# tridivb/attention_based_tbn

Hardware: AMD Instinct MI355X
Metric: clips/sec (3-seg RGB+Flow+Audio TBN fwd+bwd) (higher is better)
Workload: dtype f32; 1 GPU; BASELINE config 4: RGB+Flow+Audio async, attention off, 3 segments, 224x224 frames + 1.279 s (256x256) spectrogram, train step fwd+loss+bwd+clip+SGD; batch_per_gpu=32, global_batch=32, segments=3, parallelism=single, launch_plans=committed (bench_plans.json)

## Files before the change

### attention_based_tbn_amd/_lib.py

```python
import ctypes as C
import os

_HERE = os.path.dirname(os.path.abspath(__file__))
LIB_PATH = os.path.join(_HERE, "libtbn_hip.so")
if os.environ.get("TBN_LIB"):
    import sys as _sys
    LIB_PATH = os.path.abspath(os.environ["TBN_LIB"])
    print(f"[tbn] TBN_LIB set: loading {LIB_PATH} instead of the shipped libtbn_hip.so", file=_sys.stderr)

c_fp = C.c_void_p
c_i = C.c_int
c_sz = C.c_size_t
c_f = C.c_float


class ConvInfo(C.Structure):
    _fields_ = [("name", C.c_char * 64), ("cin", c_i), ("cout", c_i), ("ksize", c_i), ("stride", c_i),
                ("pad", c_i), ("weight_offset", c_sz), ("channel_offset", c_sz)]


class BackboneParams(C.Structure):
    _fields_ = [("weight", c_fp), ("bias", c_fp), ("gamma", c_fp), ("beta", c_fp), ("running_mean", c_fp),
                ("running_var", c_fp), ("momentum", c_f), ("eps", c_f), ("side_stream", c_fp), ("flags", c_i),
                ("weight_planes", c_fp)]
# ... 83 lines not shown
    "tbn_bn_relu_train_bwd": (c_i, [c_fp, c_i, c_fp, c_i, c_i, c_fp, c_fp, c_fp, c_fp, c_fp, c_fp, c_fp, c_fp, c_fp]),
    "tbn_bn_relu_maxpool_train_fwd": (c_i, [c_fp, c_i, c_i, c_i, c_i, c_fp, c_fp, c_fp, c_fp, c_f, c_f, c_fp, c_fp, c_fp,
                                            c_fp, c_fp, c_i, c_fp, c_i, c_i, c_i, c_i, c_fp, c_fp]),
    "tbn_bn_relu_maxpool_train_bwd": (c_i, [c_fp, c_i, c_fp, c_fp, c_i, c_i, c_i, c_i, c_i, c_i, c_i, c_i, c_fp, c_fp,
                                            c_fp, c_fp, c_fp, c_fp, c_fp, c_fp, c_fp]),
    "tbn_maxpool3_fwd": (c_i, [c_fp, c_i, c_fp, c_i, c_fp] + [c_i] * 8 + [c_fp]),
    "tbn_maxpool3_bwd": (c_i, [c_fp, c_i, c_fp, c_fp, c_i] + [c_i] * 9 + [c_fp]),
    "tbn_avgpool3_fwd": (c_i, [c_fp, c_i, c_fp, c_i] + [c_i] * 5 + [c_fp]),
    "tbn_spatial_mean_fwd": (c_i, [c_fp, c_i, c_fp, c_i] + [c_i] * 5 + [c_fp]),
    "tbn_spatial_mean_bwd": (c_i, [c_fp, c_i, c_fp, c_i] + [c_i] * 5 + [c_fp]),
    "tbn_pe_concat_fwd": (c_i, [c_fp, c_i, c_fp, c_fp, c_i, c_i, c_i, c_i, c_i, c_fp]),
    "tbn_groupnorm_fwd": (c_i, [c_fp, c_fp, c_fp, c_fp, c_fp, c_fp, c_i, c_i, c_i, c_i, c_f, c_fp]),
    "tbn_groupnorm_bwd": (c_i, [c_fp] * 8 + [c_i] * 4 + [c_fp]),
    "tbn_colsum": (c_i, [c_fp, c_i, c_fp, c_i, c_i, c_fp]),
    "tbn_mha_q1_fwd": (c_i, [c_fp] * 6 + [c_i] * 4 + [c_f, c_fp]),
    "tbn_mha_q1_bwd": (c_i, [c_fp] * 8 + [c_i] * 4 + [c_f, c_fp]),
    "tbn_weighted_sum_fwd": (c_i, [c_fp, c_fp, c_fp, c_i, c_i, c_i, c_i, c_fp]),
    "tbn_weighted_sum_bwd": (c_i, [c_fp, c_i, c_fp, c_fp, c_i, c_i, c_i, c_fp]),
    "tbn_segment_mean_fwd": (c_i, [c_fp, c_fp, c_i, c_i, c_i, c_fp]),
    "tbn_segment_mean_bwd": (c_i, [c_fp, c_fp, c_i, c_i, c_i, c_fp]),
    "tbn_dropout_fwd": (c_i, [c_fp, c_fp, c_f, c_fp, c_fp, c_sz, c_fp]),
    "tbn_ce_heads_fwd": (c_i, [c_fp, c_i, c_i, c_i, C.POINTER(c_i), C.POINTER(c_i), C.POINTER(C.c_void_p), c_fp, c_fp, c_fp, c_fp]),
    "tbn_ce_heads_bwd": (c_i, [c_fp, c_i, c_i, c_i, C.POINTER(c_i), C.POINTER(c_i), c_fp, c_fp, c_fp]),
    "tbn_mul_mask": (c_i, [c_fp, c_fp, c_fp, c_sz, c_fp]),
    "tbn_relu_mask_bwd": (c_i, [c_fp, c_fp, c_fp, c_fp, c_sz, c_fp]),
    "tbn_stft_twiddle_floats": (c_sz, []),
    "tbn_stft_make_twiddle": (c_i, [c_fp]),
    "tbn_stft_logpower": (c_i, [c_fp, c_i, c_i, c_fp, c_fp, c_f, c_fp]),
    "tbn_opt_num_partials": (c_i, [C.POINTER(OptTensor), c_i]),
    "tbn_opt_sqnorm_partials": (c_i, [C.POINTER(OptTensor), c_i, c_fp, c_fp]),
    "tbn_opt_clip_coef": (c_i, [c_fp, c_i, c_f, c_fp, c_fp, c_fp]),
    "tbn_opt_scale_grads": (c_i, [C.POINTER(OptTensor), c_i, c_fp, c_fp]),
    "tbn_opt_sgd_step": (c_i, [C.POINTER(OptTensor), c_i, c_f, c_f, c_f, c_fp, c_fp]),
    "tbn_topk_correct": (c_i, [c_fp, c_i, c_fp, c_i, c_i, c_i, c_fp, c_fp, c_fp, c_fp]),
    "tbn_frames_to_tensor": (c_i, [c_fp] + [c_i] * 16 + [c_fp, c_fp, c_i, c_i, c_fp, c_fp]),
}

_lib = None


class TbnHipError(RuntimeError):
    pass


def lib():
    global _lib
# ... 47 lines not shown
```

### attention_based_tbn_amd/core/models/model.py

```python
import os
import weakref
from collections import OrderedDict

import numpy as np
import torch
import torch.nn as nn
from torch.distributions import Categorical

from ... import ops
from .attention import MultiheadedAttention, PositionalEncoding, PrototypeAttention, UniModalAttention
from .bn_inception import bninception


class _ArenaCatFn(torch.autograd.Function):

    @staticmethod
    def forward(ctx, arena, *feats):
        ctx.widths = [f.shape[1] for f in feats]
        return arena.detach()

    @staticmethod
    def backward(ctx, g):
        out, o = [], 0
        for w in ctx.widths:
# ... 46 lines not shown
        return ops.group_norm(y.view(R, T, -1), gn.weight, gn.bias, gn.num_groups, gn.eps)

    def forward(self, x):
        return self.forward_sequence(x.squeeze(2).transpose(1, 2).contiguous()).transpose(1, 2)


class TBNModel(nn.Module):
    IN_CHANNELS = {"RGB": 3, "Flow": 10, "Audio": 1}

    def __init__(self, cfg, modality, device, pretrained_state=None):
        super().__init__()
        self.cfg = cfg
        self.modality = modality
        self.base_model_name = cfg.model.arch
        self.num_classes = cfg.model.num_classes
        self.use_attention = cfg.model.attention.enable
        self.attention_type = cfg.model.attention.type
        self.device = device
        self._pretrained_state = pretrained_state
        self.multi_stream = True
        self._streams = {}
        self.high_priority_modalities = ("Audio",)
        self.flip_weights_early = True
        self.shared_streams = {}
        if cfg.model.agg_type.lower() == "avg":
            self.agg_type = "avg"
        else:
            print("Incorrect aggregation type")
            self.agg_type = None

        in_features = 0
        for m in self.modality:
            self.add_module("Base_{}".format(m), self._create_base_model(m))
            in_features += getattr(self, "Base_{}".format(m)).feature_size
            getattr(self, "Base_{}".format(m)).use_aux_stream = len(self.modality) == 1
            getattr(self, "Base_{}".format(m)).use_branch_streams = len(self.modality) == 1
            getattr(self, "Base_{}".format(m)).stem_wgrad_last = len(self.modality) > 1
            if cfg.model.freeze_base:
                self._freeze_base_model(m, freeze_mode=cfg.model.freeze_mode)

        if len(self.modality) > 1:
            att = cfg.model.attention
            if self.use_attention and not att.use_fixed:
                attn_win_size = round(self.cfg.data.audio.audio_length * (25 / 4))
                if att.use_pe:
                    self.pe = _PEStack(PositionalEncoding(10, max_len=attn_win_size, device=device),
# ... 92 lines not shown
    def _run_backbones_inner(self, input):
        def run(m):
            b, n, c, h, w = input[m].shape
            base = getattr(self, "Base_{}".format(m))
            x = input[m].reshape(b * n, c, h, w)
            return base.forward_sequence(x) if (m == "Audio" and self.use_attention) else base(x)

        first = input[self.modality[0]]
        if not (self.multi_stream and first.is_cuda and len(self.modality) > 1):
            return {m: run(m) for m in self.modality}
        main = torch.cuda.current_stream()
        raw = {}
        share = self.shared_streams
        for m in self.modality:
            if m in share and share[m] in self._streams:
                self._streams[m] = self._streams[share[m]]
            st = self._streams.get(m)
            if st is None or st.device != first.device:
                st = self._streams[m] = torch.cuda.Stream(device=first.device,
                                                          priority=(-1 if m in self.high_priority_modalities else 0))
            st.wait_stream(main)
            with torch.cuda.stream(st):
                raw[m] = run(m)
        for m in self.modality:
            main.wait_stream(self._streams[m])
            raw[m].record_stream(main)
        if self.flip_weights_early and torch.is_grad_enabled():
            for m in self.modality:
                with torch.cuda.stream(self._streams[m]):
                    getattr(self, "Base_{}".format(m)).flip_weights_early()
        return raw

    def forward(self, input):
        features = []
        att_wts = None
        att = self.cfg.model.attention
        self._audio_dropped = False
        raw_all = self._run_backbones(input)
        for m_no, m in enumerate(self.modality):
            b, n, c, h, w = input[m].shape
            if m == "Audio":
                raw = raw_all[m]
                if (self.training and len(self.modality) > 1 and self.cfg.data.audio.dropout > 0
                        and np.random.uniform() > self.cfg.data.audio.dropout):
                    feature = torch.zeros_like(features[0])
                    self._audio_dropped = True
                elif self.use_attention:
                    seq = raw
                    if att.use_fixed:
                        feature = ops.weighted_sum(seq, input["weights"].reshape(b * n, -1).to(seq.device))
                    elif self.attention_type == "mha":
                        seq = self.pe.forward_sequence(seq)
                        feature, att_wts = self.attention_layer.attend(features[0], seq)
                        att_wts = att_wts.unsqueeze(1)
                    elif self.attention_type in ["unimodal", "proto"]:
                        feature, att_wts = self.attention_layer.attend(features[0], seq)
                else:
                    feature = raw
                if m_no > 0 and features[0].shape[0] > feature.shape[0]:
                    new_size = features[0].shape[0] // feature.shape[0]
                    feature = feature.repeat(new_size, 1)
                    n *= new_size
            else:
                feature = raw_all[m]
            features.extend([feature])
        if len(features) > 1:
            features = _concat_features(self._arena, features)
        else:
            features = features[0]
        self._arena = None

        if len(self.modality) > 1:
            features = self.fusion(features)

        out = self.classifier(features, consensus=(b, n))

        if self.use_attention and not att.use_fixed and len(self.modality) > 1:
            if att_wts is None:
                raise UnboundLocalError("local variable 'att_wts' referenced before assignment (audio dropout with a "
                                        "trainable attention layer: the reference fails the same way)")
            out["weights"] = att_wts
        return out

    def _fused_cross_entropy(self, criterion, target, preds):
        ce = criterion.get("crossentropy")
        keys = list(target["class"].keys())
        if (type(ce) is not nn.CrossEntropyLoss or ce.weight is not None or ce.ignore_index != -100
                or ce.reduction != "mean" or getattr(ce, "label_smoothing", 0.0) != 0.0 or not 1 <= len(keys) <= 4):
            return None
        shared = self.classifier.shared_scores(preds, keys)
        if shared is None:
            return None
        base, heads = shared
        labels = []
        for k in keys:
            lab = target["class"][k]
            if (not base.is_cuda or not torch.is_tensor(lab) or not lab.is_cuda or lab.dtype != torch.int64 or lab.dim() != 1
                    or lab.shape[0] != base.shape[0]):
                return None
            labels.append(lab)
        return dict(zip(keys, ops.cross_entropy_heads(base, heads, labels)))

    def get_loss(self, criterion, target, preds, epoch=0):
        assert isinstance(target, dict)
        assert isinstance(preds, dict)
        assert isinstance(criterion, dict)
        att = self.cfg.model.attention
        loss = {"total": 0, "all_class": 0}
        fused = self._fused_cross_entropy(criterion, target, preds) if hasattr(self, "classifier") else None
        for key in target["class"].keys():
            labels = target["class"][key]
            batch_size = target["class"][key].shape[0]
            loss[key] = fused[key] if fused is not None else criterion["crossentropy"](preds[key], labels)
            loss["all_class"] += loss[key]
        loss["total"] += loss["all_class"]

        if self.use_attention and not att.use_fixed:
            if self.training and epoch + 1 < att.decay_step:
                prior_multiplier = contrast_multiplier = entropy_multiplier = 0
            else:
                prior_multiplier = att.wt_decay
                contrast_multiplier = att.contrast_decay
                entropy_multiplier = att.entropy_decay
# ... 20 lines not shown
class Fusion(nn.Module):

    def __init__(self, in_size, out_size, dropout=0):
        super().__init__()
        self.in_size, self.out_size, self.dropout = in_size, out_size, dropout
        self.fusion_layer = nn.Sequential(nn.Linear(in_size, out_size), nn.ReLU())
        torch.nn.init.normal_(self.fusion_layer[0].weight, 0, 1e-3)
        torch.nn.init.constant_(self.fusion_layer[0].bias, 0)
        if self.dropout > 0:
            self.dropout_layer = nn.Dropout(p=self.dropout)

    def forward(self, input):
        lin = self.fusion_layer[0]
        out = ops.linear(input, lin.weight, lin.bias, relu=True)
        return ops.dropout(out, self.dropout, self.training)


class Classifier(nn.Module):

    def __init__(self, num_classes, in_features):
        super().__init__()
        self.num_classes = num_classes
        self._wcache, self._bcache = {}, {}
        for cls in num_classes.keys():
            self.add_module(cls, nn.Linear(in_features, self.num_classes[cls]))
            torch.nn.init.normal_(getattr(self, cls).weight, 0, 1e-3)
            torch.nn.init.constant_(getattr(self, cls).bias, 0)

    def forward(self, input, consensus=None):
        keys = list(self.num_classes.keys())
        w = ops.cat_pad_rows(self._wcache, 32, *[getattr(self, k).weight for k in keys])
        b = ops.cat_pad_rows(self._bcache, 32, *[getattr(self, k).bias for k in keys])
        scores = ops.linear(input, w, b)
        if consensus is not None:
            scores = ops.segment_mean(scores, consensus[0], consensus[1])
        out = OrderedDict()
        layout = {}
        o = 0
        for k in keys:
            out[k] = scores[:, o:o + self.num_classes[k]].contiguous()
            layout[k] = (weakref.ref(out[k]), o, self.num_classes[k], out[k]._version)
            o += self.num_classes[k]
        self._shared = (scores, layout)
        return out

    def shared_scores(self, preds, keys):
        shared = getattr(self, "_shared", None)
        if shared is None:
            return None
        scores, layout = shared
        heads = []
        for k in keys:
            ent = layout.get(k)
            t = preds.get(k) if hasattr(preds, "get") else None
            if ent is None or t is None or ent[0]() is not t or t._version != ent[3] or not scores.is_contiguous():
                return None
            heads.append((ent[1], ent[2]))
        return scores, heads
```

### attention_based_tbn_amd/csrc/api.hip

```cpp
#include <cstdarg>
#include <cstdio>
#include <cstdlib>
#include <cstring>

#include "tbn_common.h"
#include "tbn_kernels.h"
#include "../../include/tbn_hip.h"

static thread_local char g_err[512] = "";

void tbn_set_error(const char* fmt, ...) {
  va_list ap;
  va_start(ap, fmt);
  vsnprintf(g_err, sizeof(g_err), fmt, ap);
  va_end(ap);
}

#if TBN_EXPERIMENT
int tbn_env_int(const char* name, int def, int lo, int hi) {
  const char* e = getenv(name);
  if (e == nullptr || *e == 0) return def;
  char* end = nullptr;
  const long v = strtol(e, &end, 10);
  if (end == e || *end != 0 || v < lo || v > hi) {
// ... 208 lines not shown
  g_prof_open = -1;
}

__global__ __launch_bounds__(256) void mfma_burst_kernel(float* sink, int iters) {
  f32x16 a0, a1, a2, a3;
#pragma unroll
  for (int e = 0; e < 16; ++e) a0[e] = a1[e] = a2[e] = a3[e] = 0.f;
  const float x = 1e-3f * (float)(threadIdx.x & 63) + 0.5f, y = 1.0f - 1e-3f * (float)(threadIdx.x >> 6);
  for (int i = 0; i < iters; ++i) {
#pragma unroll
    for (int k = 0; k < 4; ++k) {
      a0 = __builtin_amdgcn_mfma_f32_32x32x2f32(x, y, a0, 0, 0, 0);
      a1 = __builtin_amdgcn_mfma_f32_32x32x2f32(y, x, a1, 0, 0, 0);
      a2 = __builtin_amdgcn_mfma_f32_32x32x2f32(x, x, a2, 0, 0, 0);
      a3 = __builtin_amdgcn_mfma_f32_32x32x2f32(y, y, a3, 0, 0, 0);
    }
  }
  float s = 0.f;
#pragma unroll
  for (int e = 0; e < 16; ++e) s += (a0[e] + a1[e]) + (a2[e] + a3[e]);
  if (s == -1.2345f) sink[0] = s;
}

extern "C" {

int tbn_version(void) { return 102 | (TBN_EXPERIMENT ? 0x10000 : 0); }

int tbn_capabilities(void) { return TBN_CAP_CONV_BF16X | TBN_CAP_CONV_BF16X_PLANES; }

int tbn_diag_mfma_burst(float* sink, int workgroups, int iters, double* flops, void* stream) {
  TBN_REQUIRE(sink != nullptr && workgroups > 0 && workgroups <= 65536 && iters > 0, "diag_mfma_burst: bad argument");
  hipLaunchKernelGGL(mfma_burst_kernel, dim3(workgroups), dim3(256), 0, (hipStream_t)stream, sink, iters);
  TBN_CHECK_LAUNCH("mfma_burst");
  if (flops) *flops = (double)workgroups * 4.0 * (double)iters * 16.0 * 4096.0;
  return TBN_OK;
}

int tbn_profile_enable(int on) {
  std::lock_guard<std::mutex> lk(g_prof_mu);
  g_prof_on = on != 0;
  g_prof_layers = on == 2;
  return TBN_OK;
}
int tbn_profile_reset(void) {
  std::lock_guard<std::mutex> lk(g_prof_mu);
  prof_collect();
// ... 64 lines not shown
                        float* stat_partial, int mt, int nt, void* stream) {
  ConvP p;
  conv_geom(&p, n, h, w, cin, cout, ksize, stride, pad);
  p.in = in;
  p.in_ld = in_ld;
  p.wt = weight;
  p.bias = bias;
  p.stat_partial = stat_partial;
  p.mode = epilogue;
  p.flags = flags;
  p.nseg = 1;
  p.seg[0].ptr = out;
  p.seg[0].ld = out_ld;
  p.seg[0].col_begin = 0;
  return tbn_launch_conv(p, 0, mt, nt, (hipStream_t)stream);
}

int tbn_conv2d_dgrad(const float* dout, int dout_ld, const float* weight, float* din, int din_ld, int n, int h, int w,
                     int cin, int cout, int ksize, int stride, int pad, int accumulate, float* workspace,
                     void* stream) {
  TBN_REQUIRE(dout && weight && din && workspace, "conv2d_dgrad: null pointer");
  hipStream_t st = (hipStream_t)stream;
  TBN_TRY(tbn_launch_weight_flip_transpose(weight, workspace, cout, ksize * ksize, cin, st));
  const int oh = (h + 2 * pad - ksize) / stride + 1, ow = (w + 2 * pad - ksize) / stride + 1;
  ConvP p;
  memset(&p, 0, sizeof(p));
  p.in = dout;
  p.in_ld = dout_ld;
  p.wt = workspace;
  p.N = n;
  p.H = oh;
  p.W = ow;
  p.OH = h;
  p.OW = w;
  p.Cin = cout;
  p.Cout = cin;
  p.R = p.S = ksize;
  p.stride = 1;
  p.pad = ksize - 1 - pad;
  p.up = stride;
  p.M = n * h * w;
  p.K = ksize * ksize * cout;
  p.mode = CONV_EPI_PLAIN;
  p.flags = accumulate ? CONV_FLAG_ACCUM : 0;
  p.nseg = 1;
  p.seg[0].ptr = din;
  p.seg[0].ld = din_ld;
  p.seg[0].col_begin = 0;
  return tbn_launch_conv(p, 0, 0, 0, st);
}

static int desc_to_convp(const tbn_conv_desc* d, float* workspace, hipStream_t st, ConvP* pp) {
  ConvP& p = *pp;
  TBN_REQUIRE(d && d->in && d->weight && d->out, "conv_launch: null pointer");
  if (!d->dgrad) {
    TBN_REQUIRE(d->epilogue >= 0 && d->epilogue <= 2, "conv_launch: bad epilogue");
    TBN_REQUIRE(d->epilogue != CONV_EPI_STATS || d->stat_partial, "conv_launch: stats epilogue needs stat_partial");
    TBN_REQUIRE(d->epilogue != CONV_EPI_EVAL || (d->scale && d->shift), "conv_launch: eval epilogue needs scale/shift");
    TBN_REQUIRE(d->nred == 0, "conv_launch: the fused BN-backward reduce belongs to a data gradient");
    conv_geom(&p, d->n, d->h, d->w, d->cin, d->cout, d->ksize, d->stride, d->pad);
    p.in = d->in;
    p.in_ld = d->in_ld;
    p.wt = d->weight;
    p.bias = d->bias;
    p.scale = d->scale;
    p.shift = d->shift;
    p.stat_partial = d->stat_partial;
    p.mode = d->epilogue;
  } else {
    if (d->flags & (CONV_FLAG_BF16X6 | CONV_FLAG_BF16X3 | CONV_FLAG_BF16X_PLANES)) {
      tbn_set_error("conv_launch: the bf16x kernels (flags 32 / 64) compute forward convolutions only, not dgrad = 1");
      return TBN_ERR_UNSUPPORTED;
    }
// ... 138 lines not shown
int tbn_linear_fwd(const float* x, int x_ld, const float* w, const float* bias, float* out, int out_ld, int m, int k,
                   int n, int relu, void* stream) {
  ProfPrefix scope("linear: ");
  return tbn_conv2d_fwd(x, x_ld, w, bias, out, out_ld, m, 1, 1, k, n, 1, 1, 0, CONV_EPI_PLAIN,
                        relu ? CONV_FLAG_RELU : 0, nullptr, nullptr, nullptr, stream);
}

int tbn_linear_dgrad(const float* dy, int dy_ld, const float* w, float* dx, int dx_ld, int m, int k, int n,
                     int accumulate, float* workspace, void* stream) {
  ProfPrefix scope("linear: ");
  return tbn_conv2d_dgrad(dy, dy_ld, w, dx, dx_ld, m, 1, 1, k, n, 1, 1, 0, accumulate, workspace, stream);
}

size_t tbn_linear_wgrad_workspace_floats(int m, int k, int n) { return tbn_wgrad_workspace_floats(m, n, k, 1); }

int tbn_linear_wgrad(const float* dy, int dy_ld, const float* x, int x_ld, float* dw, float* dbias, int m, int k,
                     int n, float* workspace, void* stream) {
  ProfPrefix scope("linear: ");
  TBN_TRY(tbn_conv2d_wgrad(dy, dy_ld, x, x_ld, dw, m, 1, 1, k, n, 1, 1, 0, workspace, stream));
  if (dbias) TBN_TRY(tbn_colsum(dy, dy_ld, dbias, m, n, stream));
  return TBN_OK;
}

size_t tbn_bn_workspace_floats(int p, int c) { return (size_t)tbn_bn_stats_parts(p, c) * 2 * c + 3 * (size_t)c; }

int tbn_bn_relu_train_fwd(const float* y, int p, int c, const float* gamma, const float* beta, float* running_mean,
                          float* running_var, float momentum, float eps, float* save_mean, float* save_rstd,
                          float* scale, float* shift, float* z, int z_ld, float* workspace, void* stream) {
  hipStream_t st = (hipStream_t)stream;
  int parts = 0;
  TBN_TRY(tbn_launch_bn_stats(y, c, p, c, workspace, &parts, st));
  TBN_TRY(tbn_launch_bn_finalize(workspace, parts, p, c, gamma, beta, nullptr, running_mean, running_var, momentum, eps,
                                 save_mean, save_rstd, scale, shift, st));
  Seg s;
  s.ptr = z;
  s.ld = z_ld;
  s.col_begin = 0;
  return tbn_launch_bn_apply(y, p, c, scale, shift, &s, 1, st);
}

int tbn_bn_relu_train_bwd(const float* dz, int dz_ld, const float* y, int p, int c, const float* save_mean,
                          const float* save_rstd, const float* scale, const float* shift, float* dy, float* dgamma,
                          float* dbeta, float* workspace, void* stream) {
  hipStream_t st = (hipStream_t)stream;
  CSeg s;
  s.ptr = dz;
// ... 65 lines not shown
```

### attention_based_tbn_amd/csrc/heads.hip

```cpp
#include "tbn_common.h"
#include "../../include/tbn_hip.h"

static inline int ew_grid(size_t items) {
  size_t g = (items + 255) / 256;
  return (int)(g > 4096 ? 4096 : (g < 1 ? 1 : g));
}

__device__ __forceinline__ float wave_sum(float v) {
#pragma unroll
  for (int o = 32; o > 0; o >>= 1) v += __shfl_xor(v, o);
  return v;
}

__global__ __launch_bounds__(256) void pe_concat_kernel(const float* __restrict__ feat, int feat_ld,
                                                        const float* __restrict__ pe, float* __restrict__ out,
                                                        int out_ld, int R, int T, int C, int PD) {
  const size_t total = (size_t)R * T * out_ld;
  for (size_t i = (size_t)blockIdx.x * 256 + threadIdx.x; i < total; i += (size_t)gridDim.x * 256) {
    const int c = (int)(i % out_ld);
    const size_t row = i / out_ld;
    const int t = (int)(row % T);
    float v = 0.f;
    if (c < C)
      v = feat[row * feat_ld + c];
// ... 361 lines not shown
                                                           float* __restrict__ loss) {
  const int h = blockIdx.x;
  if (h >= nheads) return;
  double acc = 0.0;
  int valid = 0;
  for (int b = threadIdx.x; b < B; b += 64) {
    acc += (double)rowloss[h * B + b];
    valid += hd.label[h][b] != -100 ? 1 : 0;
  }
  for (int o = 32; o > 0; o >>= 1) {
    acc += __shfl_xor(acc, o);
    valid += __shfl_xor(valid, o);
  }
  if (threadIdx.x == 0) loss[h] = (float)(acc / (double)valid);
}
__global__ __launch_bounds__(256) void ce_heads_bwd_kernel(const float* __restrict__ dsc, int ld, CeHeads hd, int B,
                                                           const float* __restrict__ upstream, float* __restrict__ out) {
  const int h = blockIdx.x / B, b = blockIdx.x - h * B;
  const float g = upstream[h];
  const size_t o = (size_t)b * ld + hd.col0[h];
  for (int c = threadIdx.x; c < hd.ncls[h]; c += 256) out[o + c] = dsc[o + c] * g;
}

extern "C" {

int tbn_dropout_fwd(const float* x, const float* rnd, float p, float* y, float* mask, size_t count, void* stream) {
  TBN_REQUIRE(x && rnd && y && mask && p >= 0.f && p < 1.f, "dropout_fwd: bad argument (p = %g)", (double)p);
  TBN_KLAUNCH(dropout_fwd_kernel, dim3(ew_grid(count)), dim3(256), 0, (hipStream_t)stream, x, rnd, p, 1.f / (1.f - p), y,
              mask, count);
  TBN_CHECK_LAUNCH("dropout_fwd");
  return TBN_OK;
}

int tbn_ce_heads_fwd(const float* scores, int ld, int batch, int num_heads, const int* col0, const int* ncls,
                     const long long* const* labels, float* rowloss, float* loss, float* dscores, void* stream) {
  TBN_REQUIRE(scores && col0 && ncls && labels && rowloss && loss && dscores, "ce_heads_fwd: null argument");
  TBN_REQUIRE(num_heads >= 1 && num_heads <= 4 && batch >= 1, "ce_heads_fwd: 1..4 heads, batch >= 1");
  CeHeads hd;
  hd.n = num_heads;
  for (int h = 0; h < num_heads; ++h) {
    TBN_REQUIRE(col0[h] >= 0 && ncls[h] >= 1 && col0[h] + ncls[h] <= ld && labels[h] != nullptr,
                "ce_heads_fwd: head %d covers columns [%d, %d) of %d", h, col0[h], col0[h] + ncls[h], ld);
    hd.col0[h] = col0[h];
    hd.ncls[h] = ncls[h];
    hd.label[h] = labels[h];
  }
// ... 141 lines not shown
```

### attention_based_tbn_amd/csrc/tbn_kernels.h

```cpp
#pragma once
#include "tbn_common.h"
#include <hip/hip_ext.h>

enum { CONV_EPI_PLAIN = 0, CONV_EPI_STATS = 1, CONV_EPI_EVAL = 2 };
enum {
  CONV_FLAG_ACCUM = 1,
  CONV_FLAG_RELU = 2,
  CONV_FLAG_HALO = 4,
  CONV_FLAG_DMA = 8,
  CONV_FLAG_SK4 = 16,
  CONV_FLAG_BF16X6 = 32,
  CONV_FLAG_BF16X3 = 64,
  CONV_FLAG_BF16X_PLANES = 128,
  CONV_FLAG_DESC_OUT2 = 256
};

#define TBN_CONV_MAXSEG 4
struct RedSeg {
  const float* y;
  float* partial;
  const float* stats;
  int y_ld, col_begin, C, c_off;
  unsigned y_bytes;
};
// ... 204 lines not shown
                             const float* shift, const float* mean, const float* rstd, float* partial, hipStream_t st);
int tbn_launch_bn_bwd_finalize(const float* partial, int nparts, int P, int C, const float* scale, const float* mean,
                               const float* rstd, float* coef, float* dgamma, float* dbeta, float* dbias,
                               hipStream_t st);
int tbn_launch_bn_bwd_apply(const CSeg* dz, int nseg, const float* y, int P, int C, const float* scale,
                            const float* shift, const float* coef, float* dy, hipStream_t st);

int tbn_launch_maxpool_fwd(const float* in, int in_ld, float* out, int out_ld, uint8_t* argmax, int N, int H, int W,
                           int C, int OH, int OW, int stride, int pad, hipStream_t st);
int tbn_launch_maxpool_bwd(const float* dout, int dout_ld, const uint8_t* argmax, float* din, int din_ld, int N,
                           int H, int W, int C, int OH, int OW, int stride, int pad, int accumulate, hipStream_t st);
int tbn_launch_avgpool3_fwd(const float* in, int in_ld, float* out, int out_ld, int N, int H, int W, int C,
                            int accumulate, hipStream_t st);
int tbn_launch_spatial_mean_fwd(const float* in, int in_ld, float* out, int out_ld, int N, int H, int W, int C,
                                int freq_only, hipStream_t st);
int tbn_launch_spatial_mean_bwd(const float* dout, int dout_ld, float* din, int din_ld, int N, int H, int W, int C,
                                int freq_only, hipStream_t st);
int tbn_launch_nchw_to_s2d_pad(const float* in, float* out, int N, int C, int H, int W, hipStream_t st);
int tbn_launch_pack_stem_weight_s2d(const float* w, float* wp, int Cout, int C, hipStream_t st);
int tbn_launch_unpack_stem_wgrad_s2d(const float* dwp, float* dw, int Cout, int C, hipStream_t st);
int tbn_launch_nchw_to_nhwc_pad(const float* in, float* out, int N, int C, int H, int W, int HP, int WP, hipStream_t st);
int tbn_launch_pack_stem_weight_rows(const float* w, float* wp, int Cout, int C, int RL, int K, hipStream_t st);
int tbn_launch_unpack_stem_wgrad_rows(const float* dwp, float* dw, int Cout, int C, int RL, hipStream_t st);
```

### attention_based_tbn_amd/ops.py

```python
import torch

from ._lib import call, lib, ptr, stream_ptr, TbnHipError


def _need_cuda(t, what):
    if not t.is_cuda:
        raise TbnHipError(f"{what}: tensor is on {t.device}; the TBN hot path only runs on an MI355X "
                          "(HIP) device -- there is no CPU fallback")


def _f32c(t):
    t = t.contiguous()
    if t.dtype != torch.float32:
        t = t.float()
    return t


def _pad_rows(w, b, mult):
    n = w.shape[0]
    npad = (n + mult - 1) // mult * mult
    if npad == n:
        return w, b, n
    w = torch.cat([w, w.new_zeros(npad - n, w.shape[1])], 0)
    if b is not None:
# ... 330 lines not shown
        call("tbn_ce_heads_fwd", ptr(scores), ld, B, H, col0, ncls, lptr, ptr(rowloss), ptr(loss), ptr(dsc), stream_ptr())
        ctx.heads = heads
        ctx.save_for_backward(dsc)
        return tuple(loss[h] for h in range(H))

    @staticmethod
    def backward(ctx, *grads):
        import ctypes as C
        (dsc,) = ctx.saved_tensors
        B, ld = dsc.shape
        H = len(ctx.heads)
        up = torch.stack([g if g is not None else dsc.new_zeros(()) for g in grads]).float().contiguous()
        col0 = (C.c_int * H)(*[h[0] for h in ctx.heads])
        ncls = (C.c_int * H)(*[h[1] for h in ctx.heads])
        out = torch.zeros_like(dsc)
        call("tbn_ce_heads_bwd", ptr(dsc), ld, B, H, col0, ncls, ptr(up), ptr(out), stream_ptr())
        return (out, None) + (None,) * H


def cross_entropy_heads(scores, heads, labels):
    return _CeHeadsFn.apply(scores, tuple(heads), *labels)


def dropout_mask(shape, p, training, device):
    if not training or p <= 0:
        return None
    return (torch.rand(shape, device=device) >= p).float() / (1.0 - p)
```

### include/tbn_hip.h

```cpp
#ifndef TBN_HIP_H
#define TBN_HIP_H
#include <stddef.h>
#include <stdint.h>
#ifdef __cplusplus
extern "C" {
#endif

#define TBN_ERR_ARG (-1)
#define TBN_ERR_LAUNCH (-2)
#define TBN_ERR_UNSUPPORTED (-3)

int tbn_version(void);
#define TBN_CAP_CONV_BF16X 1
#define TBN_CAP_CONV_BF16X_PLANES 2
int tbn_capabilities(void);
const char* tbn_last_error(void);

int tbn_profile_enable(int on);
int tbn_profile_reset(void);
int tbn_profile_num_entries(void);
int tbn_profile_entry(int i, char* name, int name_len, long* launches, double* total_ms, double* total_flops);
int tbn_profile_entry_bytes(int i, double* total_alg_bytes);
int tbn_diag_mfma_burst(float* sink, int workgroups, int iters, double* flops, void* stream);

// ... 162 lines not shown
int tbn_pe_concat_fwd(const float* feat, int feat_ld, const float* pe, float* out, int out_ld, int r, int t, int c,
                      int pe_dim, void* stream);
int tbn_groupnorm_fwd(const float* x, float* y, const float* gamma, const float* beta, float* save_mean,
                      float* save_rstd, int r, int t, int c, int groups, float eps, void* stream);
int tbn_groupnorm_bwd(const float* dy, const float* x, const float* gamma, const float* save_mean,
                      const float* save_rstd, float* dx, float* dgamma_part, float* dbeta_part, int r, int t, int c,
                      int groups, void* stream);
int tbn_colsum(const float* x, int x_ld, float* out, int rows, int cols, void* stream);
int tbn_mha_q1_fwd(const float* q, const float* kv, const float* drop_mask, float* ctx, float* probs, float* avg_w,
                   int r, int t, int e, int heads, float scale, void* stream);
int tbn_mha_q1_bwd(const float* dctx, const float* davg_w, const float* q, const float* kv, const float* probs,
                   const float* drop_mask, float* dq, float* dkv, int r, int t, int e, int heads, float scale,
                   void* stream);
int tbn_weighted_sum_fwd(const float* feat, const float* w, float* out, int out_ld, int r, int t, int c, void* stream);
int tbn_weighted_sum_bwd(const float* dout, int dout_ld, const float* w, float* dfeat, int r, int t, int c,
                         void* stream);
int tbn_segment_mean_fwd(const float* x, float* out, int b, int n, int c, void* stream);
int tbn_segment_mean_bwd(const float* dout, float* dx, int b, int n, int c, void* stream);
int tbn_dropout_fwd(const float* x, const float* rnd, float p, float* y, float* mask, size_t count, void* stream);
int tbn_ce_heads_fwd(const float* scores, int ld, int batch, int num_heads, const int* col0, const int* ncls,
                     const long long* const* labels, float* rowloss, float* loss, float* dscores, void* stream);
int tbn_ce_heads_bwd(const float* dscores, int ld, int batch, int num_heads, const int* col0, const int* ncls,
                     const float* upstream, float* out, void* stream);
int tbn_mul_mask(const float* x, const float* mask, float* y, size_t count, void* stream);
int tbn_relu_mask_bwd(const float* dy, const float* y, const float* mask, float* dx, size_t count, void* stream);

size_t tbn_stft_twiddle_floats(void);
int tbn_stft_make_twiddle(float* host_buffer);
int tbn_stft_logpower(const float* wave, int nseg, int len, const float* twiddle, float* spec, float eps,
                      void* stream);

#define TBN_OPT_MAX_TENSORS 48
typedef struct tbn_opt_tensor {
  void* param;
  const void* grad;
  void* momentum;
  size_t count;
} tbn_opt_tensor;
int tbn_opt_num_partials(const tbn_opt_tensor* tensors, int num_tensors);
int tbn_opt_sqnorm_partials(const tbn_opt_tensor* tensors, int num_tensors, float* partials, void* stream);
int tbn_opt_clip_coef(const float* partials, int num_partials, float max_norm, float* total_norm, float* coef,
                      void* stream);
int tbn_opt_scale_grads(const tbn_opt_tensor* tensors, int num_tensors, const float* coef, void* stream);
int tbn_opt_sgd_step(const tbn_opt_tensor* tensors, int num_tensors, float lr, float momentum, float weight_decay,
                     const float* grad_scale, void* stream);
int tbn_topk_correct(const float* scores, int scores_ld, const long long* target, int batch, int classes, int k,
// ... 12 lines not shown
```

Baseline: 900.0 clips/s.

## Fuse fusion MLP, classifier heads, consensus and loss into one head path

Adds a fused training head that runs fusion linear, dropout, classifier linear and segment consensus through one C entry point. The weight flips for backward are prepared while the backbones run on their side streams. Backward is split into a data pass and a deferred parameter-gradient pass, and CE backward writes per-row gradients directly. The aim is fewer Python autograd nodes, kernel launches and intermediate tensors in the small head, at the cost of a sizable new code path with custom gradient plumbing.

```diff
diff --git a/attention_based_tbn_amd/_lib.py b/attention_based_tbn_amd/_lib.py
--- a/attention_based_tbn_amd/_lib.py
+++ b/attention_based_tbn_amd/_lib.py
@@ -129,6 +129,13 @@
     "tbn_dropout_fwd": (c_i, [c_fp, c_fp, c_f, c_fp, c_fp, c_sz, c_fp]),
     "tbn_ce_heads_fwd": (c_i, [c_fp, c_i, c_i, c_i, C.POINTER(c_i), C.POINTER(c_i), C.POINTER(C.c_void_p), c_fp, c_fp, c_fp, c_fp]),
     "tbn_ce_heads_bwd": (c_i, [c_fp, c_i, c_i, c_i, C.POINTER(c_i), C.POINTER(c_i), c_fp, c_fp, c_fp]),
+    "tbn_head_train_fwd": (c_i, [c_fp, c_i, c_fp, c_fp, c_fp, c_f, c_fp, c_fp, c_fp, c_fp, c_fp, c_fp, c_fp, c_i,
+                                 C.POINTER(c_i), C.POINTER(c_i), C.POINTER(C.c_void_p)] + [c_i] * 6 + [c_fp]),
+    "tbn_head_ce_bwd_rows": (c_i, [c_fp, c_i, c_i, c_i, c_i, C.POINTER(c_i), C.POINTER(c_i), C.POINTER(C.c_void_p), c_fp,
+                                   c_fp]),
+    "tbn_head_flip_weights": (c_i, [c_fp, c_fp, c_fp, c_fp, c_i, c_i, c_i, c_fp]),
+    "tbn_head_bwd_data": (c_i, [c_fp, c_i, c_fp, c_fp, c_fp, c_fp, c_fp, c_fp, c_i, c_i, c_i, c_i, c_fp]),
+    "tbn_head_bwd_params": (c_i, [c_fp, c_i, c_fp, c_fp, c_fp, c_i] + [c_fp] * 6 + [c_i, c_i, c_i, c_fp]),
     "tbn_mul_mask": (c_i, [c_fp, c_fp, c_fp, c_sz, c_fp]),
     "tbn_relu_mask_bwd": (c_i, [c_fp, c_fp, c_fp, c_fp, c_sz, c_fp]),
     "tbn_stft_twiddle_floats": (c_sz, []),
diff --git a/attention_based_tbn_amd/core/models/model.py b/attention_based_tbn_amd/core/models/model.py
--- a/attention_based_tbn_amd/core/models/model.py
+++ b/attention_based_tbn_amd/core/models/model.py
@@ -92,6 +92,9 @@
         self._streams = {}
         self.high_priority_modalities = ("Audio",)
         self.flip_weights_early = True
+        self.fused_head = True
+        self._head_cache = {}
+        self._head = None
         self.shared_streams = {}
         if cfg.model.agg_type.lower() == "avg":
             self.agg_type = "avg"
@@ -230,6 +233,8 @@
             st.wait_stream(main)
             with torch.cuda.stream(st):
                 raw[m] = run(m)
+        if self._head is not None:
+            self._head.prepare_weights()
         for m in self.modality:
             main.wait_stream(self._streams[m])
             raw[m].record_stream(main)
@@ -244,7 +249,17 @@
         att_wts = None
         att = self.cfg.model.attention
         self._audio_dropped = False
-        raw_all = self._run_backbones(input)
+        self._head = token = None
+        if self._use_fused_head(input):
+            self._head = ops.FusedHead(self._head_cache, self.fusion.fusion_layer[0],
+                                       [getattr(self.classifier, k) for k in self.num_classes.keys()],
+                                       self.classifier._wcache, self.classifier._bcache, self.fusion.dropout)
+            token = self._head.token()
+        try:
+            raw_all = self._run_backbones(input)
+        except BaseException:
+            self._head = None
+            raise
         for m_no, m in enumerate(self.modality):
             b, n, c, h, w = input[m].shape
             if m == "Audio":
@@ -278,10 +293,13 @@
             features = features[0]
         self._arena = None
 
-        if len(self.modality) > 1:
-            features = self.fusion(features)
-
-        out = self.classifier(features, consensus=(b, n))
+        head, self._head = self._head, None
+        if head is not None:
+            out = self.classifier.forward_fused(head, token, features, consensus=(b, n))
+        else:
+            if len(self.modality) > 1:
+                features = self.fusion(features)
+            out = self.classifier(features, consensus=(b, n))
 
         if self.use_attention and not att.use_fixed and len(self.modality) > 1:
             if att_wts is None:
@@ -289,6 +307,14 @@
                                         "trainable attention layer: the reference fails the same way)")
             out["weights"] = att_wts
         return out
+
+    def _use_fused_head(self, input):
+        first = input[self.modality[0]]
+        if any(getattr(self, "Base_{}".format(m)).grad_bucket_fn is not None for m in self.modality):
+            return False
+        return (self.fused_head and self.training and torch.is_grad_enabled() and len(self.modality) > 1
+                and not self.use_attention and self.agg_type == "avg" and torch.is_tensor(first) and first.is_cuda
+                and 1 <= len(self.num_classes) <= 4)
 
     def _fused_cross_entropy(self, criterion, target, preds):
         ce = criterion.get("crossentropy")
@@ -307,6 +333,9 @@
                     or lab.shape[0] != base.shape[0]):
                 return None
             labels.append(lab)
+        fused = self.classifier._fused
+        if fused is not None and fused[1] is base:
+            return dict(zip(keys, ops.fused_head_loss(fused[0], base, heads, fused[2], labels)))
         return dict(zip(keys, ops.cross_entropy_heads(base, heads, labels)))
 
     def get_loss(self, criterion, target, preds, epoch=0):
@@ -373,6 +402,7 @@
         super().__init__()
         self.num_classes = num_classes
         self._wcache, self._bcache = {}, {}
+        self._fused = None
         for cls in num_classes.keys():
             self.add_module(cls, nn.Linear(in_features, self.num_classes[cls]))
             torch.nn.init.normal_(getattr(self, cls).weight, 0, 1e-3)
@@ -393,6 +423,23 @@
             layout[k] = (weakref.ref(out[k]), o, self.num_classes[k], out[k]._version)
             o += self.num_classes[k]
         self._shared = (scores, layout)
+        self._fused = None
+        return out
+
+    def forward_fused(self, head, token, input, consensus):
+        keys = list(self.num_classes.keys())
+        heads, o = [], 0
+        for k in keys:
+            heads.append((o, self.num_classes[k]))
+            o += self.num_classes[k]
+        rows, outs = ops.fused_head_forward(head, token, input, heads, consensus[0], consensus[1])
+        out = OrderedDict()
+        layout = {}
+        for k, h, t in zip(keys, heads, outs):
+            out[k] = t
+            layout[k] = (weakref.ref(t), h[0], h[1], t._version)
+        self._shared = (head.scores, layout)
+        self._fused = (rows, head.scores, consensus[1])
         return out
 
     def shared_scores(self, preds, keys):
diff --git a/attention_based_tbn_amd/csrc/api.hip b/attention_based_tbn_amd/csrc/api.hip
--- a/attention_based_tbn_amd/csrc/api.hip
+++ b/attention_based_tbn_amd/csrc/api.hip
@@ -254,6 +254,9 @@
   if (s == -1.2345f) sink[0] = s;
 }
 
+static int conv2d_dgrad_flipped(const float* dout, int dout_ld, const float* flipped, float* din, int din_ld, int n, int h,
+                                int w, int cin, int cout, int ksize, int stride, int pad, int accumulate, hipStream_t st);
+
 extern "C" {
 
 int tbn_version(void) { return 102 | (TBN_EXPERIMENT ? 0x10000 : 0); }
@@ -364,12 +367,19 @@
   TBN_REQUIRE(dout && weight && din && workspace, "conv2d_dgrad: null pointer");
   hipStream_t st = (hipStream_t)stream;
   TBN_TRY(tbn_launch_weight_flip_transpose(weight, workspace, cout, ksize * ksize, cin, st));
+  return conv2d_dgrad_flipped(dout, dout_ld, workspace, din, din_ld, n, h, w, cin, cout, ksize, stride, pad, accumulate, st);
+}
+
+}
+
+static int conv2d_dgrad_flipped(const float* dout, int dout_ld, const float* flipped, float* din, int din_ld, int n, int h,
+                                int w, int cin, int cout, int ksize, int stride, int pad, int accumulate, hipStream_t st) {
   const int oh = (h + 2 * pad - ksize) / stride + 1, ow = (w + 2 * pad - ksize) / stride + 1;
   ConvP p;
   memset(&p, 0, sizeof(p));
   p.in = dout;
   p.in_ld = dout_ld;
-  p.wt = workspace;
+  p.wt = flipped;
   p.N = n;
   p.H = oh;
   p.W = ow;
@@ -391,6 +401,8 @@
   p.seg[0].col_begin = 0;
   return tbn_launch_conv(p, 0, 0, 0, st);
 }
+
+extern "C" {
 
 static int desc_to_convp(const tbn_conv_desc* d, float* workspace, hipStream_t st, ConvP* pp) {
   ConvP& p = *pp;
@@ -575,6 +587,51 @@
   return TBN_OK;
 }
 
+int tbn_head_train_fwd(const float* x, int x_ld, const float* w_fusion, const float* b_fusion, const float* rnd, float p,
+                       float* hidden, float* mask, float* dropped, const float* w_cls, const float* b_cls, float* rows,
+                       float* scores, int num_heads, const int* col0, const int* ncls, float* const* outs, int m, int k,
+                       int hid, int ld, int b, int n, void* stream) {
+  TBN_REQUIRE(x && w_fusion && hidden && dropped && w_cls && rows && scores, "head_train_fwd: null pointer");
+  TBN_REQUIRE(m == b * n && m >= 1 && k >= 1 && hid >= 1 && ld >= 1, "head_train_fwd: m = %d is not b * n = %d * %d", m, b, n);
+  TBN_REQUIRE(p >= 0.f && p < 1.f && (p > 0.f ? (rnd && mask && dropped != hidden) : dropped == hidden),
+              "head_train_fwd: p = %g needs rnd, mask and a buffer of its own for the dropped activations; p = 0 none",
+              (double)p);
+  TBN_TRY(tbn_linear_fwd(x, x_ld, w_fusion, b_fusion, hidden, hid, m, k, hid, 1, stream));
+  if (p > 0.f) TBN_TRY(tbn_dropout_fwd(hidden, rnd, p, dropped, mask, (size_t)m * hid, stream));
+  TBN_TRY(tbn_linear_fwd(dropped, hid, w_cls, b_cls, rows, ld, m, hid, ld, 0, stream));
+  return tbn_launch_head_consensus(rows, scores, num_heads, col0, ncls, outs, b, n, ld, (hipStream_t)stream);
+}
+
+int tbn_head_ce_bwd_rows(const float* dscores, int ld, int batch, int n, int num_heads, const int* col0, const int* ncls,
+                         const float* const* upstream, float* drows, void* stream) {
+  return tbn_launch_ce_heads_bwd_rows(dscores, ld, batch, n, num_heads, col0, ncls, upstream, drows, (hipStream_t)stream);
+}
+
+int tbn_head_flip_weights(const float* w_fusion, const float* w_cls, float* wt_fusion, float* wt_cls, int k, int hid, int ld,
+                          void* stream) {
+  TBN_REQUIRE(w_fusion && w_cls && wt_fusion && wt_cls, "head_flip_weights: null pointer");
+  TBN_TRY(tbn_launch_weight_flip_transpose(w_cls, wt_cls, ld, 1, hid, (hipStream_t)stream));
+  return tbn_launch_weight_flip_transpose(w_fusion, wt_fusion, hid, 1, k, (hipStream_t)stream);
+}
+
+int tbn_head_bwd_data(const float* drows, int ld, const float* wt_cls, const float* hidden, const float* mask, float* dhidden,
+                      const float* wt_fusion, float* dx, int dx_ld, int m, int k, int hid, void* stream) {
+  TBN_REQUIRE(drows && wt_cls && hidden && dhidden && wt_fusion && dx, "head_bwd_data: null pointer");
+  ProfPrefix scope("linear: ");
+  hipStream_t st = (hipStream_t)stream;
+  TBN_TRY(conv2d_dgrad_flipped(drows, ld, wt_cls, dhidden, hid, m, 1, 1, hid, ld, 1, 1, 0, 0, st));
+  TBN_TRY(tbn_relu_mask_bwd(dhidden, hidden, mask, dhidden, (size_t)m * hid, stream));
+  return conv2d_dgrad_flipped(dhidden, hid, wt_fusion, dx, dx_ld, m, 1, 1, k, hid, 1, 1, 0, 0, st);
+}
+
+int tbn_head_bwd_params(const float* drows, int ld, const float* dropped, const float* dhidden, const float* x, int x_ld,
+                        float* dw_cls, float* db_cls, float* dw_fusion, float* db_fusion, float* ws_cls, float* ws_fusion,
+                        int m, int k, int hid, void* stream) {
+  TBN_REQUIRE(drows && dropped && dhidden && x && dw_cls && dw_fusion, "head_bwd_params: null pointer");
+  TBN_TRY(tbn_linear_wgrad(drows, ld, dropped, hid, dw_cls, db_cls, m, hid, ld, ws_cls, stream));
+  return tbn_linear_wgrad(dhidden, hid, x, x_ld, dw_fusion, db_fusion, m, k, hid, ws_fusion, stream);
+}
+
 size_t tbn_bn_workspace_floats(int p, int c) { return (size_t)tbn_bn_stats_parts(p, c) * 2 * c + 3 * (size_t)c; }
 
 int tbn_bn_relu_train_fwd(const float* y, int p, int c, const float* gamma, const float* beta, float* running_mean,
diff --git a/attention_based_tbn_amd/csrc/heads.hip b/attention_based_tbn_amd/csrc/heads.hip
--- a/attention_based_tbn_amd/csrc/heads.hip
+++ b/attention_based_tbn_amd/csrc/heads.hip
@@ -1,4 +1,5 @@
 #include "tbn_common.h"
+#include "tbn_kernels.h"
 #include "../../include/tbn_hip.h"
 
 static inline int ew_grid(size_t items) {
@@ -407,6 +408,89 @@
   for (int c = threadIdx.x; c < hd.ncls[h]; c += 256) out[o + c] = dsc[o + c] * g;
 }
 
+struct HeadOuts {
+  int n;
+  int col0[4], ncls[4];
+  float* out[4];
+};
+__global__ __launch_bounds__(256) void head_consensus_kernel(const float* __restrict__ rows, float* __restrict__ scores,
+                                                             HeadOuts ho, int B, int N, int C) {
+  const size_t total = (size_t)B * C;
+  for (size_t i = (size_t)blockIdx.x * 256 + threadIdx.x; i < total; i += (size_t)gridDim.x * 256) {
+    const int c = (int)(i % C);
+    const size_t b = i / C;
+    float s = 0.f;
+    for (int n = 0; n < N; ++n) s += rows[(b * N + n) * C + c];
+    const float v = s / (float)N;
+    scores[i] = v;
+    for (int h = 0; h < ho.n; ++h)
+      if (c >= ho.col0[h] && c < ho.col0[h] + ho.ncls[h]) ho.out[h][b * ho.ncls[h] + (c - ho.col0[h])] = v;
+  }
+}
+
+struct CeUp {
+  const float* up[4];
+};
+__global__ __launch_bounds__(256) void ce_heads_bwd_rows_kernel(const float* __restrict__ dsc, int ld, CeHeads hd, CeUp up,
+                                                                int B, int N, float* __restrict__ drows) {
+  const size_t total = (size_t)B * N * ld;
+  const float k = 1.f / (float)N;
+  for (size_t i = (size_t)blockIdx.x * 256 + threadIdx.x; i < total; i += (size_t)gridDim.x * 256) {
+    const int c = (int)(i % ld);
+    const size_t b = i / ld / N;
+    float v = 0.f;
+    for (int h = 0; h < hd.n; ++h)
+      if (c >= hd.col0[h] && c < hd.col0[h] + hd.ncls[h]) {
+        const float g = up.up[h] ? *up.up[h] : 0.f;
+        const float scaled = dsc[b * ld + c] * g;
+        v = scaled * k;
+      }
+    drows[i] = v;
+  }
+}
+
+int tbn_launch_head_consensus(const float* rows, float* scores, int num_heads, const int* col0, const int* ncls,
+                              float* const* outs, int b, int n, int ld, hipStream_t st) {
+  TBN_REQUIRE(rows && scores && col0 && ncls && outs && num_heads >= 1 && num_heads <= 4 && b >= 1 && n >= 1 && ld >= 1,
+              "head_consensus: bad argument");
+  HeadOuts ho;
+  ho.n = num_heads;
+  for (int h = 0; h < num_heads; ++h) {
+    TBN_REQUIRE(col0[h] >= 0 && ncls[h] >= 1 && col0[h] + ncls[h] <= ld && outs[h] != nullptr,
+                "head_consensus: head %d covers columns [%d, %d) of %d", h, col0[h], col0[h] + ncls[h], ld);
+    ho.col0[h] = col0[h];
+    ho.ncls[h] = ncls[h];
+    ho.out[h] = outs[h];
+  }
+  TBN_KLAUNCH(head_consensus_kernel, dim3(ew_grid((size_t)b * ld)), dim3(256), 0, st, rows, scores, ho, b, n, ld);
+  TBN_CHECK_LAUNCH("head_consensus");
+  return TBN_OK;
+}
+
+int tbn_launch_ce_heads_bwd_rows(const float* dscores, int ld, int batch, int n, int num_heads, const int* col0,
+                                 const int* ncls, const float* const* upstream, float* drows, hipStream_t st) {
+  TBN_REQUIRE(dscores && col0 && ncls && upstream && drows && num_heads >= 1 && num_heads <= 4 && batch >= 1 && n >= 1,
+              "ce_heads_bwd_rows: bad argument");
+  CeHeads hd;
+  CeUp up;
+  hd.n = num_heads;
+  for (int h = 0; h < 4; ++h) {
+    hd.col0[h] = hd.ncls[h] = 0;
+    hd.label[h] = nullptr;
+    up.up[h] = nullptr;
+  }
+  for (int h = 0; h < num_heads; ++h) {
+    TBN_REQUIRE(col0[h] >= 0 && ncls[h] >= 1 && col0[h] + ncls[h] <= ld, "ce_heads_bwd_rows: head %d out of range", h);
+    hd.col0[h] = col0[h];
+    hd.ncls[h] = ncls[h];
+    up.up[h] = upstream[h];
+  }
+  TBN_KLAUNCH(ce_heads_bwd_rows_kernel, dim3(ew_grid((size_t)batch * n * ld)), dim3(256), 0, st, dscores, ld, hd, up, batch,
+              n, drows);
+  TBN_CHECK_LAUNCH("ce_heads_bwd_rows");
+  return TBN_OK;
+}
+
 extern "C" {
 
 int tbn_dropout_fwd(const float* x, const float* rnd, float p, float* y, float* mask, size_t count, void* stream) {
diff --git a/attention_based_tbn_amd/csrc/tbn_kernels.h b/attention_based_tbn_amd/csrc/tbn_kernels.h
--- a/attention_based_tbn_amd/csrc/tbn_kernels.h
+++ b/attention_based_tbn_amd/csrc/tbn_kernels.h
@@ -250,3 +250,8 @@
 int tbn_launch_nchw_to_nhwc_pad(const float* in, float* out, int N, int C, int H, int W, int HP, int WP, hipStream_t st);
 int tbn_launch_pack_stem_weight_rows(const float* w, float* wp, int Cout, int C, int RL, int K, hipStream_t st);
 int tbn_launch_unpack_stem_wgrad_rows(const float* dwp, float* dw, int Cout, int C, int RL, hipStream_t st);
+
+int tbn_launch_head_consensus(const float* rows, float* scores, int num_heads, const int* col0, const int* ncls,
+                              float* const* outs, int b, int n, int ld, hipStream_t st);
+int tbn_launch_ce_heads_bwd_rows(const float* dscores, int ld, int batch, int n, int num_heads, const int* col0,
+                                 const int* ncls, const float* const* upstream, float* drows, hipStream_t st);
diff --git a/attention_based_tbn_amd/ops.py b/attention_based_tbn_amd/ops.py
--- a/attention_based_tbn_amd/ops.py
+++ b/attention_based_tbn_amd/ops.py
@@ -376,6 +376,205 @@
     return _CeHeadsFn.apply(scores, tuple(heads), *labels)
 
 
+class FusedHead:
+
+    def __init__(self, cache, fusion_linear, cls_linears, cls_wcache, cls_bcache, p):
+        self.cache = cache
+        self.fusion = fusion_linear
+        self.cls = list(cls_linears)
+        self.cls_wcache, self.cls_bcache = cls_wcache, cls_bcache
+        self.p = float(p)
+        self.w_cls = self.b_cls = self.wt_fusion = self.wt_cls = None
+        self.weights_key = None
+        self.scores = None
+        self.pending = None
+
+    def _key(self):
+        ps = [self.fusion.weight] + [l.weight for l in self.cls]
+        return tuple((p.data_ptr(), p._version) for p in ps)
+
+    def token(self):
+        params = [self.fusion.weight, self.fusion.bias] + [l.weight for l in self.cls] + [l.bias for l in self.cls]
+        return _HeadParamsFn.apply(self, *params)
+
+    def prepare_weights(self):
+        with torch.no_grad():
+            self.w_cls = cat_pad_rows(self.cls_wcache, 32, *[l.weight for l in self.cls])
+            self.b_cls = cat_pad_rows(self.cls_bcache, 32, *[l.bias for l in self.cls])
+        wf = self.fusion.weight
+        _need_cuda(wf, "fused head")
+        hid, k = wf.shape
+        ld = self.w_cls.shape[0]
+        bufs = self.cache.get(("wt", k, hid, ld, wf.device))
+        if bufs is None:
+            bufs = self.cache[("wt", k, hid, ld, wf.device)] = (torch.empty(k, hid, device=wf.device, dtype=torch.float32),
+                                                               torch.empty(hid, ld, device=wf.device, dtype=torch.float32))
+        self.wt_fusion, self.wt_cls = bufs
+        call("tbn_head_flip_weights", ptr(wf.detach()), ptr(self.w_cls), ptr(self.wt_fusion), ptr(self.wt_cls), k, hid, ld,
+             stream_ptr())
+        self.weights_key = self._key()
+
+    def workspaces(self, m, k, hid, ld, device):
+        key = ("ws", m, k, hid, ld, device)
+        ws = self.cache.get(key)
+        if ws is None:
+            n_cls, n_fus = lib().tbn_linear_wgrad_workspace_floats(m, hid, ld), lib().tbn_linear_wgrad_workspace_floats(m, k, hid)
+            ws = self.cache[key] = (torch.empty(max(n_cls, 1), device=device, dtype=torch.float32),
+                                    torch.empty(max(n_fus, 1), device=device, dtype=torch.float32))
+        return ws
+
+
+class _HeadParamsFn(torch.autograd.Function):
+    @staticmethod
+    def forward(ctx, head, *params):
+        ctx.set_materialize_grads(False)
+        ctx.head = head
+        return params[0].new_empty(0)
+
+    @staticmethod
+    def backward(ctx, _):
+        head = ctx.head
+        n_in = 2 + 2 * len(head.cls)
+        if head.pending is None:
+            return (None,) * (1 + n_in)
+        drows, dropped, dhidden, x = head.pending
+        head.pending = None
+        m, ld = drows.shape
+        hid, k = head.fusion.weight.shape
+        dev = drows.device
+        dw_cls = torch.empty(ld, hid, device=dev, dtype=torch.float32)
+        db_cls = torch.empty(ld, device=dev, dtype=torch.float32)
+        dw_fus = torch.empty(hid, k, device=dev, dtype=torch.float32)
+        db_fus = torch.empty(hid, device=dev, dtype=torch.float32)
+        ws_cls, ws_fus = head.workspaces(m, k, hid, ld, dev)
+        call("tbn_head_bwd_params", ptr(drows), ld, ptr(dropped), ptr(dhidden), ptr(x), x.stride(0), ptr(dw_cls), ptr(db_cls),
+             ptr(dw_fus), ptr(db_fus), ptr(ws_cls), ptr(ws_fus), m, k, hid, stream_ptr())
+        gw, gb, o = [], [], 0
+        for l in head.cls:
+            r = l.weight.shape[0]
+            gw.append(dw_cls[o:o + r])
+            gb.append(db_cls[o:o + r])
+            o += r
+        return (None, dw_fus, db_fus) + tuple(gw) + tuple(gb)
+
+
+class _HeadFn(torch.autograd.Function):
+
+    @staticmethod
+    def forward(ctx, token, x, head, heads, b, n):
+        import ctypes as C
+        _need_cuda(x, "fused head")
+        ctx.set_materialize_grads(False)
+        x = _f32c(x)
+        if head.weights_key != head._key():
+            head.prepare_weights()
+        wf, bf = head.fusion.weight.detach(), head.fusion.bias.detach()
+        m, k = x.shape
+        hid = wf.shape[0]
+        ld = head.w_cls.shape[0]
+        H = len(heads)
+        dev = x.device
+        hidden = torch.empty(m, hid, device=dev, dtype=torch.float32)
+        if head.p > 0:
+            rnd = torch.rand_like(hidden)
+            mask, dropped = torch.empty_like(hidden), torch.empty_like(hidden)
+        else:
+            rnd, mask, dropped = None, None, hidden
+        rows = torch.empty(m, ld, device=dev, dtype=torch.float32)
+        scores = torch.empty(b, ld, device=dev, dtype=torch.float32)
+        outs = [torch.empty(b, h[1], device=dev, dtype=torch.float32) for h in heads]
+        col0 = (C.c_int * H)(*[h[0] for h in heads])
+        ncls = (C.c_int * H)(*[h[1] for h in heads])
+        optr = (C.c_void_p * H)(*[o.data_ptr() for o in outs])
+        call("tbn_head_train_fwd", ptr(x), x.stride(0), ptr(wf), ptr(bf), ptr(rnd), head.p, ptr(hidden), ptr(mask),
+             ptr(dropped), ptr(head.w_cls), ptr(head.b_cls), ptr(rows), ptr(scores), H, col0, ncls, optr, m, k, hid, ld, b, n,
+             stream_ptr())
+        head.scores = scores
+        ctx.head, ctx.heads, ctx.dims = head, heads, (b, n, ld)
+        ctx.save_for_backward(x, hidden, mask, dropped)
+        return (rows,) + tuple(outs)
+
+    @staticmethod
+    def backward(ctx, drows, *douts):
+        head = ctx.head
+        x, hidden, mask, dropped = ctx.saved_tensors
+        b, n, ld = ctx.dims
+        st = stream_ptr()
+        if any(g is not None for g in douts):
+            tot = None
+            for (c0, nc), g in zip(ctx.heads, douts):
+                if g is None:
+                    continue
+                pad = g.new_zeros(b, ld)
+                pad[:, c0:c0 + nc] = g
+                tot = pad if tot is None else tot + pad
+            tot = _f32c(tot)
+            via_outs = torch.empty(b * n, ld, device=tot.device, dtype=torch.float32)
+            call("tbn_segment_mean_bwd", ptr(tot), ptr(via_outs), b, n, ld, st)
+            drows = via_outs if drows is None else drows + via_outs
+        if drows is None:
+            return (None,) * 6
+        drows = _f32c(drows)
+        if head.weights_key != head._key():
+            head.prepare_weights()
+        m, k = x.shape
+        hid = hidden.shape[1]
+        dhidden = torch.empty(m, hid, device=x.device, dtype=torch.float32)
+        dx = torch.empty(m, k, device=x.device, dtype=torch.float32)
+        call("tbn_head_bwd_data", ptr(drows), ld, ptr(head.wt_cls), ptr(hidden), ptr(mask), ptr(dhidden), ptr(head.wt_fusion),
+             ptr(dx), k, m, k, hid, st)
+        head.pending = (drows, dropped, dhidden, x)
+        return None, dx, None, None, None, None
+
+
+class _HeadLossFn(torch.autograd.Function):
+
+    @staticmethod
+    def forward(ctx, rows, scores, heads, n, *labels):
+        import ctypes as C
+        ctx.set_materialize_grads(False)
+        B, ld = scores.shape
+        H = len(heads)
+        col0 = (C.c_int * H)(*[h[0] for h in heads])
+        ncls = (C.c_int * H)(*[h[1] for h in heads])
+        labs = [l.contiguous() for l in labels]
+        for l in labs:
+            if l.dtype != torch.int64 or not l.is_cuda or l.numel() != B:
+                raise TbnHipError("fused head loss: labels must be int64 GPU tensors of the batch size")
+        lptr = (C.c_void_p * H)(*[l.data_ptr() for l in labs])
+        rowloss = torch.empty(H * B, device=scores.device, dtype=torch.float32)
+        loss = torch.empty(H, device=scores.device, dtype=torch.float32)
+        dsc = torch.empty_like(scores)
+        call("tbn_ce_heads_fwd", ptr(scores), ld, B, H, col0, ncls, lptr, ptr(rowloss), ptr(loss), ptr(dsc), stream_ptr())
+        ctx.heads, ctx.n = heads, n
+        ctx.save_for_backward(dsc)
+        return tuple(loss[h] for h in range(H))
+
+    @staticmethod
+    def backward(ctx, *grads):
+        import ctypes as C
+        (dsc,) = ctx.saved_tensors
+        B, ld = dsc.shape
+        H = len(ctx.heads)
+        ups = [None if g is None else (g if (g.dtype == torch.float32 and g.is_cuda) else g.float().to(dsc.device))
+               for g in grads]
+        col0 = (C.c_int * H)(*[h[0] for h in ctx.heads])
+        ncls = (C.c_int * H)(*[h[1] for h in ctx.heads])
+        uptr = (C.c_void_p * H)(*[ptr(u) for u in ups])
+        drows = torch.empty(B * ctx.n, ld, device=dsc.device, dtype=torch.float32)
+        call("tbn_head_ce_bwd_rows", ptr(dsc), ld, B, ctx.n, H, col0, ncls, uptr, ptr(drows), stream_ptr())
+        return (drows, None, None, None) + (None,) * H
+
+
+def fused_head_forward(head, token, x, heads, b, n):
+    res = _HeadFn.apply(token, x, head, tuple(heads), b, n)
+    return res[0], list(res[1:])
+
+
+def fused_head_loss(rows, scores, heads, n, labels):
+    return _HeadLossFn.apply(rows, scores, tuple(heads), n, *labels)
+
+
 def dropout_mask(shape, p, training, device):
     if not training or p <= 0:
         return None
diff --git a/include/tbn_hip.h b/include/tbn_hip.h
--- a/include/tbn_hip.h
+++ b/include/tbn_hip.h
@@ -208,6 +208,19 @@
                      const long long* const* labels, float* rowloss, float* loss, float* dscores, void* stream);
 int tbn_ce_heads_bwd(const float* dscores, int ld, int batch, int num_heads, const int* col0, const int* ncls,
                      const float* upstream, float* out, void* stream);
+int tbn_head_train_fwd(const float* x, int x_ld, const float* w_fusion, const float* b_fusion, const float* rnd, float p,
+                       float* hidden, float* mask, float* dropped, const float* w_cls, const float* b_cls, float* rows,
+                       float* scores, int num_heads, const int* col0, const int* ncls, float* const* outs, int m, int k,
+                       int hid, int ld, int b, int n, void* stream);
+int tbn_head_ce_bwd_rows(const float* dscores, int ld, int batch, int n, int num_heads, const int* col0, const int* ncls,
+                         const float* const* upstream, float* drows, void* stream);
+int tbn_head_flip_weights(const float* w_fusion, const float* w_cls, float* wt_fusion, float* wt_cls, int k, int hid, int ld,
+                          void* stream);
+int tbn_head_bwd_data(const float* drows, int ld, const float* wt_cls, const float* hidden, const float* mask, float* dhidden,
+                      const float* wt_fusion, float* dx, int dx_ld, int m, int k, int hid, void* stream);
+int tbn_head_bwd_params(const float* drows, int ld, const float* dropped, const float* dhidden, const float* x, int x_ld,
+                        float* dw_cls, float* db_cls, float* dw_fusion, float* db_fusion, float* ws_cls, float* ws_fusion,
+                        int m, int k, int hid, void* stream);
 int tbn_mul_mask(const float* x, const float* mask, float* y, size_t count, void* stream);
 int tbn_relu_mask_bwd(const float* dy, const float* y, const float* mask, float* dx, size_t count, void* stream);
 
```

New measurement: 901.0 clips/s (median of 2 runs). Within noise of the previous version (+0.1%).
